# pxl-th/NNop.jl

Hardware: AMD Instinct MI355X
Metric: attention TFLOPs/s + GB/s (fwd, fwd+bwd) at E=64,L=4096,H=4,B=4 (higher is better)
Workload: dtype bf16; 1 GPU; C2: bf16 non-causal flash_attention forward, E=64 L=4096 QH=4 KH=4 B=4 per GPU; per_gpu_batch=4, global_batch=4, parallelism=dp1 over (batch, kv-head) slices, step=one nnop_fa_fwd call

## Files before the change

nnop.jl_amd/_lib.py:

```python
from __future__ import annotations

import ctypes as C
import numbers
import os
import sys

_HERE = os.path.dirname(os.path.abspath(__file__))
LIB_PATH = os.environ.get("NNOP_LIB_PATH") or os.path.join(_HERE, "lib", "libnnop_hip.so")

ABI_VERSION = 7

NNOP_F32, NNOP_F16, NNOP_BF16 = 0, 1, 2

NNOP_OK = 0
NNOP_ERR_EMB_MISMATCH = -1
NNOP_ERR_KV_SHAPE = -2
NNOP_ERR_EMB_NOT_POW2 = -3
NNOP_ERR_HEADS = -4
NNOP_ERR_DTYPE = -5
NNOP_ERR_NULL = -6
NNOP_ERR_EMB_UNSUPPORTED = -7
NNOP_ERR_SHAPE = -8
NNOP_ERR_WORKSPACE = -9
NNOP_ERR_HIP = -10
NNOP_ERR_ALIGN = -11
NNOP_ERR_OPTS = -12

FWD_FORMS = {0: "fa_fwd_kernel", 1: "fa_fwd_split_kernel", 2: "fa_fwd_w64_kernel", 3: "fa_fwd_generic_kernel", 4: "fa_fwd_duo_kernel"}
FWD_FORMS_CAP = {0: "fa_fwd_cap_kernel", 3: "fa_fwd_generic_cap_kernel"}
TUNE_KEYS = {"fwd_split": 0, "fwd_nw": 1, "fwd_w64": 2, "bwd_big7": 3, "norm_bwd_cap": 4, "bwd_nw": 5,
             "fwd_exact_scale": 6, "bwd_w64": 7, "bwd_stages": 8, "fwd_persist": 9, "bwd_persist": 10, "fwd_duo": 11, "fwd_persist_asc": 12, "bwd_narrow": 13, "fwd_causal_alt": 14}


class FaShard(C.Structure):
    """struct nnop_fa_shard (declared below FaDesc; fields filled in after it)"""


class FaDesc(C.Structure):
    _fields_ = [
        ("dtype", C.c_int32), ("emb", C.c_int32), ("ql", C.c_int32), ("kl", C.c_int32),
        ("qh", C.c_int32), ("kh", C.c_int32), ("batch", C.c_int32), ("causal", C.c_int32),
        ("emb_k", C.c_int32), ("emb_v", C.c_int32), ("kl_v", C.c_int32), ("kh_v", C.c_int32),
    ]


FaShard._fields_ = [("desc", FaDesc), ("b0", C.c_int32), ("b1", C.c_int32), ("kh0", C.c_int32), ("kh1", C.c_int32),
# ... 206 lines not shown
```

nnop.jl_amd/csrc/fa_fwd.hpp:

```cpp
#pragma once
#include <type_traits>
#include "fa_common.hpp"

#if !defined(NNOP_DEV_BUILD)
#undef NNOP_ABL
#endif
#ifndef NNOP_ABL
#define NNOP_ABL 0
#endif
#if !defined(NNOP_DEV_BUILD)
#undef NNOP_V_PREFETCH
#undef NNOP_V_DEEP
#undef NNOP_V_MFMASUM
#undef NNOP_V_SETPRIO
#endif
#ifndef NNOP_V_PREFETCH
#define NNOP_V_PREFETCH 1
#endif
#ifndef NNOP_V_DEEP
#define NNOP_V_DEEP 1
#endif
#ifndef NNOP_V_MFMASUM
#define NNOP_V_MFMASUM 1
#endif
// ... 16 lines not shown
    const uint8_t* kpad;
    int   QL, KL, QH, KH, B;
    int   causal;
    int   n_qblk;
    int   n_wg;
    float scale;
    int   persist_hx = 0;
    int   persist = 0;
    int   persist_asc = 0;
    int   causal_alt = 0;
    int   win_left = -1;
    int   win_right = -1;
    const float* sinks = nullptr;
    float cap_ka = 0.f;
    float cap_kb = 0.f;
#ifdef NNOP_DEV_BUILD
    int   stagger = 0;
#endif
};

#include "fa_fwd_kernel.inc"

template <typename T, int E, int BK> constexpr int fa_fwd_lds_bytes() {
    return 2 * (RowImg<T, E>::bytes(BK) + ColImg<T, E>::bytes(BK)) + 16 + 8 * kMaxMaskTiles;
}

}
```

nnop.jl_amd/csrc/fa_fwd_duo_asm.inc:

```
#define NNOP_DUO_SLOTS_PER_GROUP 3
#define NNOP_DUO_VALU_SUMS 0
#define NNOP_DUO_SYNC_ONE 1

#define NNOP_DUO_LOOP_PLAIN(TS, MP1, MP0, VP1, VP0) \
    "v_mov_b32 v208, 0\n\t" \
    "v_mov_b32 v209, 0\n\t" \
    "v_mov_b32 v210, 0xff800000\n\t" \
    "v_mov_b32 v211, 0xff800000\n\t" \
    "s_cmp_lg_u32 %[st], 0\n\t" \
    "s_cbranch_scc1 L_loop1_%=\n\t" \
    "L_loop0_%=:\n\t" \
    "s_cmp_lt_i32 %[st], %[snlive]\n\t" \
    "s_cselect_b32 s56, 1, 0\n\t" \
    "s_sub_i32 s58, %[st], 2\n\t" \
    "s_cmp_lt_i32 s58, %[snlive]\n\t" \
    "s_cselect_b32 s57, 1, 0\n\t" \
    "s_cmp_lt_i32 s58, 0\n\t" \
    "s_cselect_b32 s57, 0, s57\n\t" \
    "v_add_u32 v204, %[ska], v199\n\t" \
    "v_add_u32 v205, %[sva], v200\n\t" \
    "s_add_i32 s58, %[st], 4\n\t" \
    "s_lshl_b32 s58, s58, 13\n\t" \
    "s_min_u32 s60, s58, %[slast]\n\t" \
    "s_add_i32 s58, %[st], 2\n\t" \
// ... 549 lines not shown
    "v_mul_f32 v58, v58, v217\n\t" \
    "v_mul_f32 v59, v59, v217\n\t" \
    "v_mul_f32 v60, v60, v217\n\t" \
    "v_mul_f32 v61, v61, v217\n\t" \
    "v_mul_f32 v62, v62, v217\n\t" \
    "v_mul_f32 v63, v63, v217\n\t" \
    "ds_bpermute_b32 v218, v212, v217\n\t" \
    "ds_bpermute_b32 v219, v213, v217\n\t" \
    "s_waitcnt lgkmcnt(0)\n\t" \
    "v_mul_f32 v100, v100, v218\n\t" \
    "v_mul_f32 v101, v101, v219\n\t" \
    "s_branch L_rescdone0_%=\n\t" \
    "L_exit0_%=:\n\t" \
    "s_branch L_end_%=\n\t" \
    "L_loop1_%=:\n\t" \
    "s_cmp_lt_i32 %[st], %[snlive]\n\t" \
    "s_cselect_b32 s56, 1, 0\n\t" \
    "s_sub_i32 s58, %[st], 2\n\t" \
    "s_cmp_lt_i32 s58, %[snlive]\n\t" \
    "s_cselect_b32 s57, 1, 0\n\t" \
    "s_cmp_lt_i32 s58, 0\n\t" \
    "s_cselect_b32 s57, 0, s57\n\t" \
    "v_add_u32 v204, %[ska], v199\n\t" \
    "v_add_u32 v205, %[sva], v200\n\t" \
    "s_add_i32 s58, %[st], 4\n\t" \
    "s_lshl_b32 s58, s58, 13\n\t" \
    "s_min_u32 s60, s58, %[slast]\n\t" \
    "s_add_i32 s58, %[st], 2\n\t" \
    "s_lshl_b32 s58, s58, 13\n\t" \
    "s_min_u32 s61, s58, %[slast]\n\t" \
// ... 547 lines not shown
    "v_mul_f32 v55, v55, v217\n\t" \
    "v_mul_f32 v56, v56, v217\n\t" \
    "v_mul_f32 v57, v57, v217\n\t" \
    "v_mul_f32 v58, v58, v217\n\t" \
    "v_mul_f32 v59, v59, v217\n\t" \
    "v_mul_f32 v60, v60, v217\n\t" \
    "v_mul_f32 v61, v61, v217\n\t" \
    "v_mul_f32 v62, v62, v217\n\t" \
    "v_mul_f32 v63, v63, v217\n\t" \
    "ds_bpermute_b32 v218, v212, v217\n\t" \
    "ds_bpermute_b32 v219, v213, v217\n\t" \
    "s_waitcnt lgkmcnt(0)\n\t" \
    "v_mul_f32 v100, v100, v218\n\t" \
    "v_mul_f32 v101, v101, v219\n\t" \
    "s_branch L_rescdone1_%=\n\t" \
    "L_exit1_%=:\n\t" \
    "L_end_%=:\n\t"

#define NNOP_DUO_LOOP_MASKED(TS, MP1, MP0, VP1, VP0) \
    "v_mov_b32 v208, 0\n\t" \
    "v_mov_b32 v209, 0\n\t" \
    "v_mov_b32 v210, 0xff800000\n\t" \
    "v_mov_b32 v211, 0xff800000\n\t" \
    "s_cmp_lg_u32 %[st], 0\n\t" \
    "s_cbranch_scc1 L_loop1_%=\n\t" \
    "L_loop0_%=:\n\t" \
    "s_cmp_lt_i32 %[st], %[snlive]\n\t" \
    "s_cselect_b32 s56, 1, 0\n\t" \
    "s_sub_i32 s58, %[st], 2\n\t" \
    "s_cmp_lt_i32 s58, %[snlive]\n\t" \
// ... 7739 lines not shown
    "v_mul_f32 v58, v58, v217\n\t" \
    "v_mul_f32 v59, v59, v217\n\t" \
    "v_mul_f32 v60, v60, v217\n\t" \
    "v_mul_f32 v61, v61, v217\n\t" \
    "v_mul_f32 v62, v62, v217\n\t" \
    "v_mul_f32 v63, v63, v217\n\t" \
    "ds_bpermute_b32 v218, v212, v217\n\t" \
    "ds_bpermute_b32 v219, v213, v217\n\t" \
    "s_waitcnt lgkmcnt(0)\n\t" \
    "v_mul_f32 v100, v100, v218\n\t" \
    "v_mul_f32 v101, v101, v219\n\t" \
    "s_branch L_rescdone0_%=\n\t" \
    "L_exit0_%=:\n\t" \
    "s_branch L_end_%=\n\t" \
    "L_loop1_%=:\n\t" \
    "s_cmp_lt_i32 %[st], %[snlive]\n\t" \
    "s_cselect_b32 s56, 1, 0\n\t" \
    "s_sub_i32 s58, %[st], 2\n\t" \
    "s_cmp_lt_i32 s58, %[snlive]\n\t" \
    "s_cselect_b32 s57, 1, 0\n\t" \
    "s_cmp_lt_i32 s58, 0\n\t" \
    "s_cselect_b32 s57, 0, s57\n\t" \
    "v_add_u32 v204, %[ska], v199\n\t" \
    "v_add_u32 v205, %[sva], v200\n\t" \
    "s_add_i32 s58, %[st], 4\n\t" \
    "s_lshl_b32 s58, s58, 13\n\t" \
    "s_min_u32 s60, s58, %[slast]\n\t" \
    "s_add_i32 s58, %[st], 2\n\t" \
    "s_lshl_b32 s58, s58, 13\n\t" \
    "s_min_u32 s61, s58, %[slast]\n\t" \
// ... 567 lines not shown
    "v_mul_f32 v55, v55, v217\n\t" \
    "v_mul_f32 v56, v56, v217\n\t" \
    "v_mul_f32 v57, v57, v217\n\t" \
    "v_mul_f32 v58, v58, v217\n\t" \
    "v_mul_f32 v59, v59, v217\n\t" \
    "v_mul_f32 v60, v60, v217\n\t" \
    "v_mul_f32 v61, v61, v217\n\t" \
    "v_mul_f32 v62, v62, v217\n\t" \
    "v_mul_f32 v63, v63, v217\n\t" \
    "ds_bpermute_b32 v218, v212, v217\n\t" \
    "ds_bpermute_b32 v219, v213, v217\n\t" \
    "s_waitcnt lgkmcnt(0)\n\t" \
    "v_mul_f32 v100, v100, v218\n\t" \
    "v_mul_f32 v101, v101, v219\n\t" \
    "s_branch L_rescdone1_%=\n\t" \
    "L_exit1_%=:\n\t" \
    "L_end_%=:\n\t" \
    "v_mov_b32 v224, s71\n\t" \
    "v_mov_b32 v225, s72\n\t" \
    "v_mov_b32 v226, s73\n\t" \
    "v_mov_b32 v227, s74\n\t" \
    "v_mov_b32 v228, s75\n\t"

#define NNOP_DUO_LOOP_MASKED_PROF(TS, MP1, MP0, VP1, VP0) \
    "v_mov_b32 v208, 0\n\t" \
    "v_mov_b32 v209, 0\n\t" \
    "v_mov_b32 v210, 0xff800000\n\t" \
    "v_mov_b32 v211, 0xff800000\n\t" \
    "s_memtime s[68:69]\n\t" \
    "s_waitcnt lgkmcnt(0)\n\t" \
// ... 1732 lines not shown
```

nnop.jl_amd/csrc/fa_fwd_duo_kernel.inc:

```
template <typename T, int E, int MODE, int NZ = 2, bool SINK = false>
__global__ __launch_bounds__(512) void fa_fwd_duo_kernel(const FwdParams p) {
    static_assert(sizeof(T) == 2 && ((E == 64 && (NZ == 1 || NZ == 2)) || (E == 128 && NZ == 1) || (E == 32 && NZ == 2)),
                  "16-bit element types; E = 64, E = 128 with 32-row waves, E = 32 with 64-row waves");
    constexpr int RW = 32 * NZ, RB = 4 * RW;
    using frag_t = typename Elem<T>::frag;
    using KImg   = RowImg<T, E>;
    using VImg   = ColImg<T, E>;
    constexpr bool kGeneral = MODE != 0;
    constexpr int BK = 64, KB = 2, KS = E / 16, EB = E / 32, NS = 2 * duo_slots_per_group<E>();
    constexpr int KBYTES = KImg::bytes(BK), VBYTES = VImg::bytes(BK);
    constexpr int RING = NS * (KBYTES + VBYTES);
    constexpr int MASK_OFF = RING > kDuoXchgBytes ? RING : kDuoXchgBytes;
    constexpr int TILE_BYTES = BK * E * (int)sizeof(T);
    constexpr int NJK = KBYTES / 4096, NJV = VBYTES / 4096;
    static_assert(NJK * 4096 == KBYTES && NJV * 4096 == VBYTES && NJK <= 4 && NJV <= 4, "four waves x NJ pieces = one image");

    extern __shared__ __attribute__((aligned(16))) char smem[];
#if NNOP_DUO_STAMP
    uint64_t stamp[8];
    stamp[0] = __builtin_amdgcn_s_memtime();
    stamp[1] = __builtin_amdgcn_s_memrealtime();
#endif
    const int tid = threadIdx.x, lane = tid & 63;
    const int wave = __builtin_amdgcn_readfirstlane(tid >> 6);
// ... 165 lines not shown

    f32x16 sc[NZ][KB];
#pragma unroll
    for (int z = 0; z < NZ; ++z)
#pragma unroll
        for (int kb = 0; kb < KB; ++kb)
#pragma unroll
            for (int i = 0; i < 16; ++i) sc[z][kb][i] = 0.f;

    f32x4 mstate = {-INFINITY, -INFINITY, -INFINITY, -INFINITY};
    typedef uint32_t u32x8 __attribute__((ext_vector_type(8)));
    u32x8 vconst;
    vconst[0] = k_voff[0]; vconst[1] = k_voff[NJK > 1 ? 1 : 0]; vconst[2] = v_voff; vconst[3] = k_lane; vconst[4] = v_lane;
    vconst[5] = (uint32_t)qlim[0]; vconst[6] = (uint32_t)qlim[1]; vconst[7] = (uint32_t)(4 * h);
    int s_t = grp, s_h = n_tiles + 2, s_nlive = n_live, s_cq0 = causal_q0;
    uint32_t s_ka = kA, s_kb = kB, s_kc = kC, s_va = vA, s_vb = vB, s_vc = vC;
    const uint32_t s_last = (uint32_t)(n_tiles - 1) * (uint32_t)TILE_BYTES, s_vbits = (uint32_t)(uintptr_t)vbits;
#if NNOP_DUO_STAMP
    f32x8 profv = {0.f, 0.f, 0.f, 0.f, 0.f, 0.f, 0.f, 0.f};
#endif
#if NNOP_DUO_VALU_SUMS
    f32x4 lsum = {0.f, 0.f, 0.f, 0.f};
#endif
#if NNOP_DUO_PRIO == 2
    if (grp) __builtin_amdgcn_s_setprio(1);
#endif
    if constexpr (!duo_sync_one<E>()) {
        if (grp) asm volatile("s_barrier" ::: "memory");
    }
#if NNOP_DUO_STAMP
// ... 175 lines not shown
```

nnop.jl_amd/csrc/fa_fwd_inst.hpp:

```cpp
#pragma once
#include "fa_fwd.hpp"
#include "fa_fwd_split.hpp"
#include "fa_fwd_w64.hpp"
#include "fa_fwd_duo.hpp"
#include "fa_generic.hpp"
#ifdef NNOP_DEV_BUILD
#include <stdlib.h>
#endif
#include "fa_launch.hpp"
#include <math.h>

namespace nnop {

#ifdef NNOP_DEV_BUILD
static inline int dev_env_int(const char* name, int dflt) {
    const char* s = getenv(name);
    return (s && *s) ? atoi(s) : dflt;
}
#endif

static inline int fwd_params(FwdParams& p, const nnop_fa_desc& d, const FwdArgs& a, int rows) {
    p = FwdParams{};
    p.o = a.o; p.ms = a.ms; p.ls = a.ls;
    p.q = a.q; p.k = a.k; p.v = a.v; p.pair = a.pair; p.kpad = a.kpad;
// ... 89 lines not shown

template <typename T, int E, int MODE, int NZ, bool SINK = false>
static int launch_fwd_duo(const nnop_fa_desc& d, const FwdArgs& a, hipStream_t s) {
    if constexpr (!SINK) {
        if (a.sinks) return launch_fwd_duo<T, E, MODE, NZ, true>(d, a, s);
    }
    constexpr int lds = fa_fwd_duo_lds_bytes<T, E>(MODE != 0);
    static_assert(lds <= 160 * 1024, "LDS budget");
    constexpr auto kern = fa_fwd_duo_kernel<T, E, MODE, NZ, SINK>;
    static unsigned long long lds_done = 0;
    if (ensure_dynamic_lds(kern, lds, &lds_done) != NNOP_OK) return NNOP_ERR_HIP;
    FwdParams p;
    if (const int st = fwd_params(p, d, a, 128 * NZ); st != NNOP_OK) return st;
    long long grid = p.n_wg;
    if constexpr (MODE == 1) fwd_persist_plan(d, a, p, grid);
    hipLaunchKernelGGL(kern, dim3((unsigned)grid), dim3(512), lds, s, p);
    return hipGetLastError() == hipSuccess ? NNOP_OK : NNOP_ERR_HIP;
}

static inline int fwd_mode(const nnop_fa_desc& d, bool has_pair, bool has_mask, bool win_on, bool capped) {
    return has_pair ? 2 : ((d.causal || has_mask || win_on || capped || (d.kl % 64) != 0) ? 1 : 0);
}
static inline long long fwd_wg(const nnop_fa_desc& d, int rows) { return (long long)((d.ql + rows - 1) / rows) * d.qh * d.batch; }
static inline bool fwd_wide_fits(const nnop_fa_desc& d, int mode) {
    return mode != 2 && (mode == 0 || d.kl <= 64 * kMaxMaskTiles) && (long long)d.kl * d.emb * 2 < (1LL << 32);
}
static inline int fwd_duo_nz(const nnop_fa_desc& d) {
    const int duo = tune_get(kTuneFwdDuo);
    if (duo == 2) return 2;
    if (duo == 3) return 1;
// ... 124 lines not shown
```

nnop.jl_amd/csrc/nnop_capi.cpp:

```cpp
#include "fa_launch.hpp"
#include "host_common.hpp"
#include "nnop_debug.h"
#include "tuning.hpp"
#include <limits.h>
#include <stdlib.h>
#include <mutex>

namespace nnop {

static int g_tune[kTuneCount];
static int g_debug_hooks = 0;
static std::once_flag g_tune_once;
static void tune_init() {
    static const char* const names[kTuneCount] = {"NNOP_FWD_SPLIT", "NNOP_FWD_NW",       "NNOP_FWD_W64",
                                                  "NNOP_BWD_BIG7",  "NNOP_NORM_BWD_CAP", "NNOP_BWD_NW",
                                                  "NNOP_FWD_EXACT_SCALE", "NNOP_BWD_W64", nullptr, "NNOP_FWD_PERSIST", "NNOP_BWD_PERSIST",
                                                  "NNOP_FWD_DUO", "NNOP_FWD_PERSIST_ASC", "NNOP_BWD_NARROW", "NNOP_FWD_CAUSAL_ALT"};
    for (int k = 0; k < kTuneCount; ++k) {
        const char* s = names[k] ? getenv(names[k]) : nullptr;
        __atomic_store_n(&g_tune[k], (s && *s) ? atoi(s) : -1, __ATOMIC_RELAXED);
    }
    const char* h = getenv("NNOP_DEBUG_HOOKS");
    __atomic_store_n(&g_debug_hooks, (h && *h && atoi(h) != 0) ? 1 : 0, __ATOMIC_RELAXED);
}
int tune_get(int key) {
    std::call_once(g_tune_once, tune_init);
    return __atomic_load_n(&g_tune[key], __ATOMIC_RELAXED);
}

static int check_desc(const nnop_fa_desc* d) {
    if (!d) return NNOP_ERR_NULL;
    if (!known_dtype(d->dtype)) return NNOP_ERR_DTYPE;
// ... 432 lines not shown
```

nnop.jl_amd/csrc/tuning.hpp:

```cpp
#pragma once

namespace nnop {

enum TuneKey {
    kTuneFwdSplit = 0,
    kTuneFwdNW,
    kTuneFwdW64,
    kTuneBwdBig7,
    kTuneNormBwdCap,
    kTuneBwdNW,
    kTuneFwdExactScale,
    kTuneBwdW64,
    kTuneBwdStages,
    kTuneFwdPersist,
    kTuneBwdPersist,
    kTuneFwdDuo,
    kTuneFwdPersistAsc,
    kTuneBwdNarrow,
    kTuneFwdCausalAlt,
    kTuneCount
};

int tune_get(int key);

}
```

Measured before the change: 1019 TFLOP/s.

## Add unrolled steady-state inner loop to duo forward attention kernel

Adds a specialized steady-state path to the duo forward kernel's main loop. For E=64 with two row groups in the unmasked mode, the loop is unrolled three times with the K/V LDS buffer rotation fixed at compile time. This drops the per-iteration liveness checks, buffer-offset computation and branching of the general loop, and moves the rare online-softmax rescale to out-of-line blocks. It is gated by a new NNOP_FWD_DUO_STEADY knob that is on by default. In exchange it adds a large amount of hand-written asm and a padded rescale path with long s_nop runs, which costs time whenever a rescale is taken.

After: 975.1 TFLOP/s. -4.3%, worse.

```diff
diff --git a/nnop.jl_amd/_lib.py b/nnop.jl_amd/_lib.py
--- a/nnop.jl_amd/_lib.py
+++ b/nnop.jl_amd/_lib.py
@@ -29,7 +29,7 @@
 FWD_FORMS = {0: "fa_fwd_kernel", 1: "fa_fwd_split_kernel", 2: "fa_fwd_w64_kernel", 3: "fa_fwd_generic_kernel", 4: "fa_fwd_duo_kernel"}
 FWD_FORMS_CAP = {0: "fa_fwd_cap_kernel", 3: "fa_fwd_generic_cap_kernel"}
 TUNE_KEYS = {"fwd_split": 0, "fwd_nw": 1, "fwd_w64": 2, "bwd_big7": 3, "norm_bwd_cap": 4, "bwd_nw": 5,
-             "fwd_exact_scale": 6, "bwd_w64": 7, "bwd_stages": 8, "fwd_persist": 9, "bwd_persist": 10, "fwd_duo": 11, "fwd_persist_asc": 12, "bwd_narrow": 13, "fwd_causal_alt": 14}
+             "fwd_exact_scale": 6, "bwd_w64": 7, "bwd_stages": 8, "fwd_persist": 9, "bwd_persist": 10, "fwd_duo": 11, "fwd_persist_asc": 12, "bwd_narrow": 13, "fwd_causal_alt": 14, "fwd_duo_steady": 15}
 
 
 class FaShard(C.Structure):
diff --git a/nnop.jl_amd/csrc/fa_fwd.hpp b/nnop.jl_amd/csrc/fa_fwd.hpp
--- a/nnop.jl_amd/csrc/fa_fwd.hpp
+++ b/nnop.jl_amd/csrc/fa_fwd.hpp
@@ -54,6 +54,7 @@
     const float* sinks = nullptr;
     float cap_ka = 0.f;
     float cap_kb = 0.f;
+    int   duo_steady = 0;
 #ifdef NNOP_DEV_BUILD
     int   stagger = 0;
 #endif
diff --git a/nnop.jl_amd/csrc/fa_fwd_duo_asm.inc b/nnop.jl_amd/csrc/fa_fwd_duo_asm.inc
--- a/nnop.jl_amd/csrc/fa_fwd_duo_asm.inc
+++ b/nnop.jl_amd/csrc/fa_fwd_duo_asm.inc
@@ -1,6 +1,437 @@
 #define NNOP_DUO_SLOTS_PER_GROUP 3
 #define NNOP_DUO_VALU_SUMS 0
 #define NNOP_DUO_SYNC_ONE 1
+
+
+#define NNOP_DUO_STEADY_COPY1(TS, MP1, MP0, VP1, VP0, C, KA, KB, KC, VA, VB, VC, T71, T73, T74, T75) \
+    "v_add_u32 v204, " KA ", v199\n\t" \
+    "v_add_u32 v205, " VA ", v200\n\t" \
+    "" MP1 "\n\t" \
+    "v_xor_b32 v108, 32, v204\n\t" \
+    "v_xor_b32 v109, 64, v204\n\t" \
+    "v_xor_b32 v110, 96, v204\n\t" \
+    "ds_read_b64_tr_b16 v[176:177], v205 offset:0\n\t" \
+    "ds_read_b64_tr_b16 v[178:179], v205 offset:1024\n\t" \
+    "ds_read_b64_tr_b16 v[180:181], v205 offset:256\n\t" \
+    "ds_read_b64_tr_b16 v[182:183], v205 offset:1280\n\t" \
+    "ds_read_b64_tr_b16 v[184:185], v205 offset:2048\n\t" \
+    "ds_read_b64_tr_b16 v[186:187], v205 offset:3072\n\t" \
+    "v_mfma_f32_16x16x32_" TS " v[96:99], v[104:107], v[112:115], v[96:99]\n\t" \
+    "v_mfma_f32_16x16x32_" TS " v[100:103], v[104:107], v[144:147], v[100:103]\n\t" \
+    "v_mfma_f32_16x16x32_" TS " v[96:99], v[104:107], v[120:123], v[96:99]\n\t" \
+    "v_mfma_f32_16x16x32_" TS " v[100:103], v[104:107], v[152:155], v[100:103]\n\t" \
+    "v_mfma_f32_16x16x32_" TS " v[96:99], v[104:107], v[128:131], v[96:99]\n\t" \
+    "v_mfma_f32_16x16x32_" TS " v[100:103], v[104:107], v[160:163], v[100:103]\n\t" \
+    "v_mfma_f32_16x16x32_" TS " v[96:99], v[104:107], v[136:139], v[96:99]\n\t" \
+    "v_mfma_f32_16x16x32_" TS " v[100:103], v[104:107], v[168:171], v[100:103]\n\t" \
+    "ds_read_b64_tr_b16 v[188:189], v205 offset:2304\n\t" \
+    "ds_read_b64_tr_b16 v[190:191], v205 offset:3328\n\t" \
+    "s_waitcnt lgkmcnt(6)\n\t" \
+    "v_mfma_f32_32x32x16_" TS " v[0:15], v[176:179], v[112:115], v[0:15]\n\t" \
+    "v_mfma_f32_32x32x16_" TS " v[32:47], v[176:179], v[144:147], v[32:47]\n\t" \
+    "ds_read_b64_tr_b16 v[176:177], v205 offset:4096\n\t" \
+    "ds_read_b64_tr_b16 v[178:179], v205 offset:5120\n\t" \
+    "s_waitcnt lgkmcnt(6)\n\t" \
+    "v_mfma_f32_32x32x16_" TS " v[16:31], v[180:183], v[112:115], v[16:31]\n\t" \
+    "v_mfma_f32_32x32x16_" TS " v[48:63], v[180:183], v[144:147], v[48:63]\n\t" \
+    "ds_read_b64_tr_b16 v[180:181], v205 offset:4352\n\t" \
+    "ds_read_b64_tr_b16 v[182:183], v205 offset:5376\n\t" \
+    "s_waitcnt lgkmcnt(6)\n\t" \
+    "v_mfma_f32_32x32x16_" TS " v[0:15], v[184:187], v[120:123], v[0:15]\n\t" \
+    "v_mfma_f32_32x32x16_" TS " v[32:47], v[184:187], v[152:155], v[32:47]\n\t" \
+    "ds_read_b64_tr_b16 v[184:185], v205 offset:6144\n\t" \
+    "ds_read_b64_tr_b16 v[186:187], v205 offset:7168\n\t" \
+    "s_waitcnt lgkmcnt(6)\n\t" \
+    "v_mfma_f32_32x32x16_" TS " v[16:31], v[188:191], v[120:123], v[16:31]\n\t" \
+    "v_mfma_f32_32x32x16_" TS " v[48:63], v[188:191], v[152:155], v[48:63]\n\t" \
+    "ds_read_b64_tr_b16 v[188:189], v205 offset:6400\n\t" \
+    "ds_read_b64_tr_b16 v[190:191], v205 offset:7424\n\t" \
+    "s_waitcnt lgkmcnt(6)\n\t" \
+    "v_mfma_f32_32x32x16_" TS " v[0:15], v[176:179], v[128:131], v[0:15]\n\t" \
+    "v_mfma_f32_32x32x16_" TS " v[32:47], v[176:179], v[160:163], v[32:47]\n\t" \
+    "ds_read_b128 v[176:179], v204 offset:0\n\t" \
+    "s_waitcnt lgkmcnt(5)\n\t" \
+    "v_mfma_f32_32x32x16_" TS " v[16:31], v[180:183], v[128:131], v[16:31]\n\t" \
+    "v_mfma_f32_32x32x16_" TS " v[48:63], v[180:183], v[160:163], v[48:63]\n\t" \
+    "ds_read_b128 v[180:183], v108 offset:0\n\t" \
+    "s_waitcnt lgkmcnt(4)\n\t" \
+    "v_mfma_f32_32x32x16_" TS " v[0:15], v[184:187], v[136:139], v[0:15]\n\t" \
+    "v_mfma_f32_32x32x16_" TS " v[32:47], v[184:187], v[168:171], v[32:47]\n\t" \
+    "ds_read_b128 v[184:187], v109 offset:0\n\t" \
+    "s_waitcnt lgkmcnt(3)\n\t" \
+    "v_mfma_f32_32x32x16_" TS " v[16:31], v[188:191], v[136:139], v[16:31]\n\t" \
+    "v_mfma_f32_32x32x16_" TS " v[48:63], v[188:191], v[168:171], v[48:63]\n\t" \
+    "ds_read_b128 v[188:191], v110 offset:0\n\t" \
+    "s_waitcnt lgkmcnt(3)\n\t" \
+    "v_mfma_f32_32x32x16_" TS " v[112:127], v[176:179], v[64:67], 0\n\t" \
+    "v_mfma_f32_32x32x16_" TS " v[144:159], v[176:179], v[80:83], 0\n\t" \
+    "ds_read_b128 v[176:179], v204 offset:4096\n\t" \
+    "s_waitcnt lgkmcnt(3)\n\t" \
+    "v_mfma_f32_32x32x16_" TS " v[112:127], v[180:183], v[68:71], v[112:127]\n\t" \
+    "v_mfma_f32_32x32x16_" TS " v[144:159], v[180:183], v[84:87], v[144:159]\n\t" \
+    "ds_read_b128 v[180:183], v108 offset:4096\n\t" \
+    "s_waitcnt lgkmcnt(3)\n\t" \
+    "v_mfma_f32_32x32x16_" TS " v[112:127], v[184:187], v[72:75], v[112:127]\n\t" \
+    "v_mfma_f32_32x32x16_" TS " v[144:159], v[184:187], v[88:91], v[144:159]\n\t" \
+    "ds_read_b128 v[184:187], v109 offset:4096\n\t" \
+    "s_waitcnt lgkmcnt(3)\n\t" \
+    "v_mfma_f32_32x32x16_" TS " v[112:127], v[188:191], v[76:79], v[112:127]\n\t" \
+    "v_mfma_f32_32x32x16_" TS " v[144:159], v[188:191], v[92:95], v[144:159]\n\t" \
+    "ds_read_b128 v[188:191], v110 offset:4096\n\t" \
+    "s_waitcnt lgkmcnt(3)\n\t" \
+    "v_mfma_f32_32x32x16_" TS " v[128:143], v[176:179], v[64:67], 0\n\t" \
+    "v_mfma_f32_32x32x16_" TS " v[160:175], v[176:179], v[80:83], 0\n\t" \
+    "s_waitcnt lgkmcnt(2)\n\t" \
+    "v_mfma_f32_32x32x16_" TS " v[128:143], v[180:183], v[68:71], v[128:143]\n\t" \
+    "v_mfma_f32_32x32x16_" TS " v[160:175], v[180:183], v[84:87], v[160:175]\n\t" \
+    "s_waitcnt lgkmcnt(1)\n\t" \
+    "v_mfma_f32_32x32x16_" TS " v[128:143], v[184:187], v[72:75], v[128:143]\n\t" \
+    "v_mfma_f32_32x32x16_" TS " v[160:175], v[184:187], v[88:91], v[160:175]\n\t" \
+    "s_waitcnt lgkmcnt(0)\n\t" \
+    "v_mfma_f32_32x32x16_" TS " v[128:143], v[188:191], v[76:79], v[128:143]\n\t" \
+    "v_mfma_f32_32x32x16_" TS " v[160:175], v[188:191], v[92:95], v[160:175]\n\t" \
+    "s_mov_b32 m0, " KC "\n\t" \
+    "s_nop 0\n\t" \
+    "buffer_load_dwordx4 v196, %[krs], s60 offen offset:0 lds\n\t" \
+    "buffer_load_dwordx4 v197, %[krs], s60 offen offset:1024 lds\n\t" \
+    "s_mov_b32 m0, " VC "\n\t" \
+    "s_nop 0\n\t" \
+    "buffer_load_dwordx4 v198, %[vrs], s61 offen offset:0 lds\n\t" \
+    "buffer_load_dwordx4 v198, %[vrs], s61 offen offset:1024 lds\n\t" \
+    "" MP0 "\n\t" \
+    "" T71 "\n\t" \
+    "" T73 "\n\t" \
+    "s_waitcnt vmcnt(4)\n\t" \
+    "" T74 "\n\t" \
+    "s_barrier\n\t" \
+    "" T75 "\n\t" \
+    "" VP1 "\n\t" \
+    "v_max_f32 v176, v112, v113\n\t" \
+    "v_max_f32 v180, v144, v145\n\t" \
+    "v_max_f32 v177, v114, v115\n\t" \
+    "v_max_f32 v181, v146, v147\n\t" \
+    "v_max_f32 v178, v116, v117\n\t" \
+    "v_max_f32 v182, v148, v149\n\t" \
+    "v_max_f32 v179, v118, v119\n\t" \
+    "v_max_f32 v183, v150, v151\n\t" \
+    "v_max3_f32 v176, v176, v120, v121\n\t" \
+    "v_max3_f32 v180, v180, v152, v153\n\t" \
+    "v_max3_f32 v177, v177, v122, v123\n\t" \
+    "v_max3_f32 v181, v181, v154, v155\n\t" \
+    "v_max3_f32 v178, v178, v124, v125\n\t" \
+    "v_max3_f32 v182, v182, v156, v157\n\t" \
+    "v_max3_f32 v179, v179, v126, v127\n\t" \
+    "v_max3_f32 v183, v183, v158, v159\n\t" \
+    "v_max3_f32 v176, v176, v128, v129\n\t" \
+    "v_max3_f32 v180, v180, v160, v161\n\t" \
+    "v_max3_f32 v177, v177, v130, v131\n\t" \
+    "v_max3_f32 v181, v181, v162, v163\n\t" \
+    "v_max3_f32 v178, v178, v132, v133\n\t" \
+    "v_max3_f32 v182, v182, v164, v165\n\t" \
+    "v_max3_f32 v179, v179, v134, v135\n\t" \
+    "v_max3_f32 v183, v183, v166, v167\n\t" \
+    "v_max3_f32 v176, v176, v136, v137\n\t" \
+    "v_max3_f32 v180, v180, v168, v169\n\t" \
+    "v_max3_f32 v177, v177, v138, v139\n\t" \
+    "v_max3_f32 v181, v181, v170, v171\n\t" \
+    "v_max3_f32 v178, v178, v140, v141\n\t" \
+    "v_max3_f32 v182, v182, v172, v173\n\t" \
+    "v_max3_f32 v179, v179, v142, v143\n\t" \
+    "v_max3_f32 v183, v183, v174, v175\n\t" \
+    "v_max3_f32 v176, v176, v177, v178\n\t" \
+    "v_max3_f32 v180, v180, v181, v182\n\t" \
+    "v_max_f32 v206, v176, v179\n\t" \
+    "v_max_f32 v207, v180, v183\n\t" \
+    "v_mul_f32 v206, %[sc2], v206\n\t" \
+    "v_mul_f32 v207, %[sc2], v207\n\t" \
+    "v_max_f32 v194, v194, v206\n\t" \
+    "v_max_f32 v195, v195, v207\n\t" \
+    "v_cmp_gt_f32 vcc, v206, v210\n\t" \
+    "v_cmp_gt_f32 s[64:65], v207, v211\n\t" \
+    "s_or_b64 s[64:65], s[64:65], vcc\n\t" \
+    "s_cbranch_scc1 L_strescale1" C "_%=\n\t" \
+    "L_strescdone1" C "_%=:\n\t" \
+    "v_fma_f32 v112, v112, %[sc2], v208\n\t" \
+    "v_fma_f32 v113, v113, %[sc2], v208\n\t" \
+    "v_fma_f32 v114, v114, %[sc2], v208\n\t" \
+    "v_fma_f32 v115, v115, %[sc2], v208\n\t" \
+    "v_fma_f32 v116, v116, %[sc2], v208\n\t" \
+    "v_exp_f32 v112, v112\n\t" \
+    "v_fma_f32 v117, v117, %[sc2], v208\n\t" \
+    "v_exp_f32 v113, v113\n\t" \
+    "v_fma_f32 v118, v118, %[sc2], v208\n\t" \
+    "v_exp_f32 v114, v114\n\t" \
+    "v_fma_f32 v119, v119, %[sc2], v208\n\t" \
+    "v_exp_f32 v115, v115\n\t" \
+    "v_fma_f32 v144, v144, %[sc2], v209\n\t" \
+    "v_exp_f32 v116, v116\n\t" \
+    "v_fma_f32 v145, v145, %[sc2], v209\n\t" \
+    "v_exp_f32 v117, v117\n\t" \
+    "v_cvt_pk_" TS "_f32 v112, v112, v113\n\t" \
+    "v_fma_f32 v146, v146, %[sc2], v209\n\t" \
+    "v_exp_f32 v118, v118\n\t" \
+    "v_fma_f32 v147, v147, %[sc2], v209\n\t" \
+    "v_exp_f32 v119, v119\n\t" \
+    "v_cvt_pk_" TS "_f32 v113, v114, v115\n\t" \
+    "v_fma_f32 v148, v148, %[sc2], v209\n\t" \
+    "v_exp_f32 v144, v144\n\t" \
+    "v_fma_f32 v149, v149, %[sc2], v209\n\t" \
+    "v_exp_f32 v145, v145\n\t" \
+    "v_cvt_pk_" TS "_f32 v114, v116, v117\n\t" \
+    "v_fma_f32 v150, v150, %[sc2], v209\n\t" \
+    "v_exp_f32 v146, v146\n\t" \
+    "v_fma_f32 v151, v151, %[sc2], v209\n\t" \
+    "v_exp_f32 v147, v147\n\t" \
+    "v_cvt_pk_" TS "_f32 v115, v118, v119\n\t" \
+    "v_fma_f32 v120, v120, %[sc2], v208\n\t" \
+    "v_exp_f32 v148, v148\n\t" \
+    "v_fma_f32 v121, v121, %[sc2], v208\n\t" \
+    "v_exp_f32 v149, v149\n\t" \
+    "v_cvt_pk_" TS "_f32 v144, v144, v145\n\t" \
+    "v_fma_f32 v122, v122, %[sc2], v208\n\t" \
+    "v_exp_f32 v150, v150\n\t" \
+    "v_fma_f32 v123, v123, %[sc2], v208\n\t" \
+    "v_exp_f32 v151, v151\n\t" \
+    "v_cvt_pk_" TS "_f32 v145, v146, v147\n\t" \
+    "v_fma_f32 v124, v124, %[sc2], v208\n\t" \
+    "v_exp_f32 v120, v120\n\t" \
+    "v_fma_f32 v125, v125, %[sc2], v208\n\t" \
+    "v_exp_f32 v121, v121\n\t" \
+    "v_cvt_pk_" TS "_f32 v146, v148, v149\n\t" \
+    "v_fma_f32 v126, v126, %[sc2], v208\n\t" \
+    "v_exp_f32 v122, v122\n\t" \
+    "v_fma_f32 v127, v127, %[sc2], v208\n\t" \
+    "v_exp_f32 v123, v123\n\t" \
+    "v_cvt_pk_" TS "_f32 v147, v150, v151\n\t" \
+    "v_fma_f32 v152, v152, %[sc2], v209\n\t" \
+    "v_exp_f32 v124, v124\n\t" \
+    "v_fma_f32 v153, v153, %[sc2], v209\n\t" \
+    "v_exp_f32 v125, v125\n\t" \
+    "v_cvt_pk_" TS "_f32 v120, v120, v121\n\t" \
+    "v_fma_f32 v154, v154, %[sc2], v209\n\t" \
+    "v_exp_f32 v126, v126\n\t" \
+    "v_fma_f32 v155, v155, %[sc2], v209\n\t" \
+    "v_exp_f32 v127, v127\n\t" \
+    "v_cvt_pk_" TS "_f32 v121, v122, v123\n\t" \
+    "v_fma_f32 v156, v156, %[sc2], v209\n\t" \
+    "v_exp_f32 v152, v152\n\t" \
+    "v_fma_f32 v157, v157, %[sc2], v209\n\t" \
+    "v_exp_f32 v153, v153\n\t" \
+    "v_cvt_pk_" TS "_f32 v122, v124, v125\n\t" \
+    "v_fma_f32 v158, v158, %[sc2], v209\n\t" \
+    "v_exp_f32 v154, v154\n\t" \
+    "v_fma_f32 v159, v159, %[sc2], v209\n\t" \
+    "v_exp_f32 v155, v155\n\t" \
+    "v_cvt_pk_" TS "_f32 v123, v126, v127\n\t" \
+    "v_fma_f32 v128, v128, %[sc2], v208\n\t" \
+    "v_exp_f32 v156, v156\n\t" \
+    "v_fma_f32 v129, v129, %[sc2], v208\n\t" \
+    "v_exp_f32 v157, v157\n\t" \
+    "v_cvt_pk_" TS "_f32 v152, v152, v153\n\t" \
+    "v_fma_f32 v130, v130, %[sc2], v208\n\t" \
+    "v_exp_f32 v158, v158\n\t" \
+    "v_fma_f32 v131, v131, %[sc2], v208\n\t" \
+    "v_exp_f32 v159, v159\n\t" \
+    "v_cvt_pk_" TS "_f32 v153, v154, v155\n\t" \
+    "v_fma_f32 v132, v132, %[sc2], v208\n\t" \
+    "v_exp_f32 v128, v128\n\t" \
+    "v_fma_f32 v133, v133, %[sc2], v208\n\t" \
+    "v_exp_f32 v129, v129\n\t" \
+    "v_cvt_pk_" TS "_f32 v154, v156, v157\n\t" \
+    "v_fma_f32 v134, v134, %[sc2], v208\n\t" \
+    "v_exp_f32 v130, v130\n\t" \
+    "v_fma_f32 v135, v135, %[sc2], v208\n\t" \
+    "v_exp_f32 v131, v131\n\t" \
+    "v_cvt_pk_" TS "_f32 v155, v158, v159\n\t" \
+    "v_fma_f32 v160, v160, %[sc2], v209\n\t" \
+    "v_exp_f32 v132, v132\n\t" \
+    "v_fma_f32 v161, v161, %[sc2], v209\n\t" \
+    "v_exp_f32 v133, v133\n\t" \
+    "v_cvt_pk_" TS "_f32 v128, v128, v129\n\t" \
+    "v_fma_f32 v162, v162, %[sc2], v209\n\t" \
+    "v_exp_f32 v134, v134\n\t" \
+    "v_fma_f32 v163, v163, %[sc2], v209\n\t" \
+    "v_exp_f32 v135, v135\n\t" \
+    "v_cvt_pk_" TS "_f32 v129, v130, v131\n\t" \
+    "v_fma_f32 v164, v164, %[sc2], v209\n\t" \
+    "v_exp_f32 v160, v160\n\t" \
+    "v_fma_f32 v165, v165, %[sc2], v209\n\t" \
+    "v_exp_f32 v161, v161\n\t" \
+    "v_cvt_pk_" TS "_f32 v130, v132, v133\n\t" \
+    "v_fma_f32 v166, v166, %[sc2], v209\n\t" \
+    "v_exp_f32 v162, v162\n\t" \
+    "v_fma_f32 v167, v167, %[sc2], v209\n\t" \
+    "v_exp_f32 v163, v163\n\t" \
+    "v_cvt_pk_" TS "_f32 v131, v134, v135\n\t" \
+    "v_fma_f32 v136, v136, %[sc2], v208\n\t" \
+    "v_exp_f32 v164, v164\n\t" \
+    "v_fma_f32 v137, v137, %[sc2], v208\n\t" \
+    "v_exp_f32 v165, v165\n\t" \
+    "v_cvt_pk_" TS "_f32 v160, v160, v161\n\t" \
+    "v_fma_f32 v138, v138, %[sc2], v208\n\t" \
+    "v_exp_f32 v166, v166\n\t" \
+    "v_fma_f32 v139, v139, %[sc2], v208\n\t" \
+    "v_exp_f32 v167, v167\n\t" \
+    "v_cvt_pk_" TS "_f32 v161, v162, v163\n\t" \
+    "v_fma_f32 v140, v140, %[sc2], v208\n\t" \
+    "v_exp_f32 v136, v136\n\t" \
+    "v_fma_f32 v141, v141, %[sc2], v208\n\t" \
+    "v_exp_f32 v137, v137\n\t" \
+    "v_cvt_pk_" TS "_f32 v162, v164, v165\n\t" \
+    "v_fma_f32 v142, v142, %[sc2], v208\n\t" \
+    "v_exp_f32 v138, v138\n\t" \
+    "v_fma_f32 v143, v143, %[sc2], v208\n\t" \
+    "v_exp_f32 v139, v139\n\t" \
+    "v_cvt_pk_" TS "_f32 v163, v166, v167\n\t" \
+    "v_fma_f32 v168, v168, %[sc2], v209\n\t" \
+    "v_exp_f32 v140, v140\n\t" \
+    "v_fma_f32 v169, v169, %[sc2], v209\n\t" \
+    "v_exp_f32 v141, v141\n\t" \
+    "v_cvt_pk_" TS "_f32 v136, v136, v137\n\t" \
+    "v_fma_f32 v170, v170, %[sc2], v209\n\t" \
+    "v_exp_f32 v142, v142\n\t" \
+    "v_fma_f32 v171, v171, %[sc2], v209\n\t" \
+    "v_exp_f32 v143, v143\n\t" \
+    "v_cvt_pk_" TS "_f32 v137, v138, v139\n\t" \
+    "v_fma_f32 v172, v172, %[sc2], v209\n\t" \
+    "v_exp_f32 v168, v168\n\t" \
+    "v_fma_f32 v173, v173, %[sc2], v209\n\t" \
+    "v_exp_f32 v169, v169\n\t" \
+    "v_cvt_pk_" TS "_f32 v138, v140, v141\n\t" \
+    "v_fma_f32 v174, v174, %[sc2], v209\n\t" \
+    "v_exp_f32 v170, v170\n\t" \
+    "v_fma_f32 v175, v175, %[sc2], v209\n\t" \
+    "v_exp_f32 v171, v171\n\t" \
+    "v_cvt_pk_" TS "_f32 v139, v142, v143\n\t" \
+    "v_exp_f32 v172, v172\n\t" \
+    "v_exp_f32 v173, v173\n\t" \
+    "v_cvt_pk_" TS "_f32 v168, v168, v169\n\t" \
+    "v_exp_f32 v174, v174\n\t" \
+    "v_exp_f32 v175, v175\n\t" \
+    "v_cvt_pk_" TS "_f32 v169, v170, v171\n\t" \
+    "v_cvt_pk_" TS "_f32 v170, v172, v173\n\t" \
+    "v_cvt_pk_" TS "_f32 v171, v174, v175\n\t" \
+    "" VP0 "\n\t" \
+    "s_add_u32 s60, s60, 16384\n\t" \
+    "s_add_u32 s61, s61, 16384\n\t"
+
+#define NNOP_DUO_RESCALE \
+    "s_nop 15\n\t" \
+    "s_nop 15\n\t" \
+    "s_nop 15\n\t" \
+    "s_nop 15\n\t" \
+    "s_nop 15\n\t" \
+    "s_nop 15\n\t" \
+    "s_nop 15\n\t" \
+    "s_nop 15\n\t" \
+    "v_mov_b32 v220, v206\n\t" \
+    "v_mov_b32 v221, v207\n\t" \
+    "s_nop 1\n\t" \
+    "v_permlane32_swap_b32 v206, v220\n\t" \
+    "v_permlane32_swap_b32 v207, v221\n\t" \
+    "v_max_f32 v206, v206, v220\n\t" \
+    "v_max_f32 v207, v207, v221\n\t" \
+    "v_mbcnt_lo_u32_b32 v214, -1, 0\n\t" \
+    "v_mbcnt_hi_u32_b32 v214, -1, v214\n\t" \
+    "v_and_b32 v212, 15, v214\n\t" \
+    "v_lshlrev_b32 v212, 2, v212\n\t" \
+    "v_add_u32 v213, 64, v212\n\t" \
+    "v_cmp_gt_f32 vcc, v206, v210\n\t" \
+    "v_cndmask_b32 v216, v192, v206, vcc\n\t" \
+    "v_sub_f32 v217, v192, v216\n\t" \
+    "v_exp_f32 v217, v217\n\t" \
+    "s_nop 0\n\t" \
+    "v_cndmask_b32 v217, 1.0, v217, vcc\n\t" \
+    "v_mov_b32 v192, v216\n\t" \
+    "v_cmp_eq_f32 vcc, 0xff800000, v216\n\t" \
+    "v_sub_f32 v208, 0, v216\n\t" \
+    "v_cndmask_b32 v208, v208, 0, vcc\n\t" \
+    "v_add_f32 v210, 0x41000000, v216\n\t" \
+    "v_mul_f32 v0, v0, v217\n\t" \
+    "v_mul_f32 v1, v1, v217\n\t" \
+    "v_mul_f32 v2, v2, v217\n\t" \
+    "v_mul_f32 v3, v3, v217\n\t" \
+    "v_mul_f32 v4, v4, v217\n\t" \
+    "v_mul_f32 v5, v5, v217\n\t" \
+    "v_mul_f32 v6, v6, v217\n\t" \
+    "v_mul_f32 v7, v7, v217\n\t" \
+    "v_mul_f32 v8, v8, v217\n\t" \
+    "v_mul_f32 v9, v9, v217\n\t" \
+    "v_mul_f32 v10, v10, v217\n\t" \
+    "v_mul_f32 v11, v11, v217\n\t" \
+    "v_mul_f32 v12, v12, v217\n\t" \
+    "v_mul_f32 v13, v13, v217\n\t" \
+    "v_mul_f32 v14, v14, v217\n\t" \
+    "v_mul_f32 v15, v15, v217\n\t" \
+    "v_mul_f32 v16, v16, v217\n\t" \
+    "v_mul_f32 v17, v17, v217\n\t" \
+    "v_mul_f32 v18, v18, v217\n\t" \
+    "v_mul_f32 v19, v19, v217\n\t" \
+    "v_mul_f32 v20, v20, v217\n\t" \
+    "v_mul_f32 v21, v21, v217\n\t" \
+    "v_mul_f32 v22, v22, v217\n\t" \
+    "v_mul_f32 v23, v23, v217\n\t" \
+    "v_mul_f32 v24, v24, v217\n\t" \
+    "v_mul_f32 v25, v25, v217\n\t" \
+    "v_mul_f32 v26, v26, v217\n\t" \
+    "v_mul_f32 v27, v27, v217\n\t" \
+    "v_mul_f32 v28, v28, v217\n\t" \
+    "v_mul_f32 v29, v29, v217\n\t" \
+    "v_mul_f32 v30, v30, v217\n\t" \
+    "v_mul_f32 v31, v31, v217\n\t" \
+    "ds_bpermute_b32 v218, v212, v217\n\t" \
+    "ds_bpermute_b32 v219, v213, v217\n\t" \
+    "s_waitcnt lgkmcnt(0)\n\t" \
+    "v_mul_f32 v96, v96, v218\n\t" \
+    "v_mul_f32 v97, v97, v219\n\t" \
+    "v_cmp_gt_f32 vcc, v207, v211\n\t" \
+    "v_cndmask_b32 v216, v193, v207, vcc\n\t" \
+    "v_sub_f32 v217, v193, v216\n\t" \
+    "v_exp_f32 v217, v217\n\t" \
+    "s_nop 0\n\t" \
+    "v_cndmask_b32 v217, 1.0, v217, vcc\n\t" \
+    "v_mov_b32 v193, v216\n\t" \
+    "v_cmp_eq_f32 vcc, 0xff800000, v216\n\t" \
+    "v_sub_f32 v209, 0, v216\n\t" \
+    "v_cndmask_b32 v209, v209, 0, vcc\n\t" \
+    "v_add_f32 v211, 0x41000000, v216\n\t" \
+    "v_mul_f32 v32, v32, v217\n\t" \
+    "v_mul_f32 v33, v33, v217\n\t" \
+    "v_mul_f32 v34, v34, v217\n\t" \
+    "v_mul_f32 v35, v35, v217\n\t" \
+    "v_mul_f32 v36, v36, v217\n\t" \
+    "v_mul_f32 v37, v37, v217\n\t" \
+    "v_mul_f32 v38, v38, v217\n\t" \
+    "v_mul_f32 v39, v39, v217\n\t" \
+    "v_mul_f32 v40, v40, v217\n\t" \
+    "v_mul_f32 v41, v41, v217\n\t" \
+    "v_mul_f32 v42, v42, v217\n\t" \
+    "v_mul_f32 v43, v43, v217\n\t" \
+    "v_mul_f32 v44, v44, v217\n\t" \
+    "v_mul_f32 v45, v45, v217\n\t" \
+    "v_mul_f32 v46, v46, v217\n\t" \
+    "v_mul_f32 v47, v47, v217\n\t" \
+    "v_mul_f32 v48, v48, v217\n\t" \
+    "v_mul_f32 v49, v49, v217\n\t" \
+    "v_mul_f32 v50, v50, v217\n\t" \
+    "v_mul_f32 v51, v51, v217\n\t" \
+    "v_mul_f32 v52, v52, v217\n\t" \
+    "v_mul_f32 v53, v53, v217\n\t" \
+    "v_mul_f32 v54, v54, v217\n\t" \
+    "v_mul_f32 v55, v55, v217\n\t" \
+    "v_mul_f32 v56, v56, v217\n\t" \
+    "v_mul_f32 v57, v57, v217\n\t" \
+    "v_mul_f32 v58, v58, v217\n\t" \
+    "v_mul_f32 v59, v59, v217\n\t" \
+    "v_mul_f32 v60, v60, v217\n\t" \
+    "v_mul_f32 v61, v61, v217\n\t" \
+    "v_mul_f32 v62, v62, v217\n\t" \
+    "v_mul_f32 v63, v63, v217\n\t" \
+    "ds_bpermute_b32 v218, v212, v217\n\t" \
+    "ds_bpermute_b32 v219, v213, v217\n\t" \
+    "s_waitcnt lgkmcnt(0)\n\t" \
+    "v_mul_f32 v100, v100, v218\n\t" \
+    "v_mul_f32 v101, v101, v219\n\t"
 
 #define NNOP_DUO_LOOP_PLAIN(TS, MP1, MP0, VP1, VP0) \
     "v_mov_b32 v208, 0\n\t" \
@@ -587,6 +1018,12 @@
     "L_exit0_%=:\n\t" \
     "s_branch L_end_%=\n\t" \
     "L_loop1_%=:\n\t" \
+    "s_cmp_lt_i32 %[st], 2\n\t" \
+    "s_cbranch_scc1 L_general1_%=\n\t" \
+    "s_add_i32 s58, %[st], 11\n\t" \
+    "s_cmp_le_i32 s58, %[scq0]\n\t" \
+    "s_cbranch_scc1 L_steady1_%=\n\t" \
+    "L_general1_%=:\n\t" \
     "s_cmp_lt_i32 %[st], %[snlive]\n\t" \
     "s_cselect_b32 s56, 1, 0\n\t" \
     "s_sub_i32 s58, %[st], 2\n\t" \
@@ -1164,6 +1601,26 @@
     "v_mul_f32 v100, v100, v218\n\t" \
     "v_mul_f32 v101, v101, v219\n\t" \
     "s_branch L_rescdone1_%=\n\t" \
+    "L_steady1_%=:\n\t" \
+    "s_add_i32 s58, %[st], 4\n\t" \
+    "s_lshl_b32 s60, s58, 13\n\t" \
+    "s_add_i32 s58, %[st], 2\n\t" \
+    "s_lshl_b32 s61, s58, 13\n\t" \
+    "L_sttrip1_%=:\n\t" \
+    NNOP_DUO_STEADY_COPY1(TS, MP1, MP0, VP1, VP0, "0", "%[ska]", "%[skb]", "%[skc]", "%[sva]", "%[svb]", "%[svc]", "", "", "", "") \
+    NNOP_DUO_STEADY_COPY1(TS, MP1, MP0, VP1, VP0, "1", "%[skb]", "%[skc]", "%[ska]", "%[svb]", "%[svc]", "%[sva]", "", "", "", "") \
+    NNOP_DUO_STEADY_COPY1(TS, MP1, MP0, VP1, VP0, "2", "%[skc]", "%[ska]", "%[skb]", "%[svc]", "%[sva]", "%[svb]", "", "", "", "") \
+    "s_add_i32 %[st], %[st], 6\n\t" \
+    "s_add_i32 s58, %[st], 11\n\t" \
+    "s_cmp_le_i32 s58, %[scq0]\n\t" \
+    "s_cbranch_scc1 L_sttrip1_%=\n\t" \
+    "s_branch L_loop1_%=\n\t" \
+    "L_strescale10_%=:\n\t" NNOP_DUO_RESCALE \
+    "s_branch L_strescdone10_%=\n\t" \
+    "L_strescale11_%=:\n\t" NNOP_DUO_RESCALE \
+    "s_branch L_strescdone11_%=\n\t" \
+    "L_strescale12_%=:\n\t" NNOP_DUO_RESCALE \
+    "s_branch L_strescdone12_%=\n\t" \
     "L_exit1_%=:\n\t" \
     "L_end_%=:\n\t"
 
@@ -8933,6 +9390,12 @@
     "L_exit0_%=:\n\t" \
     "s_branch L_end_%=\n\t" \
     "L_loop1_%=:\n\t" \
+    "s_cmp_lt_i32 %[st], 2\n\t" \
+    "s_cbranch_scc1 L_general1_%=\n\t" \
+    "s_add_i32 s58, %[st], 11\n\t" \
+    "s_cmp_le_i32 s58, %[scq0]\n\t" \
+    "s_cbranch_scc1 L_steady1_%=\n\t" \
+    "L_general1_%=:\n\t" \
     "s_cmp_lt_i32 %[st], %[snlive]\n\t" \
     "s_cselect_b32 s56, 1, 0\n\t" \
     "s_sub_i32 s58, %[st], 2\n\t" \
@@ -9530,6 +9993,26 @@
     "v_mul_f32 v100, v100, v218\n\t" \
     "v_mul_f32 v101, v101, v219\n\t" \
     "s_branch L_rescdone1_%=\n\t" \
+    "L_steady1_%=:\n\t" \
+    "s_add_i32 s58, %[st], 4\n\t" \
+    "s_lshl_b32 s60, s58, 13\n\t" \
+    "s_add_i32 s58, %[st], 2\n\t" \
+    "s_lshl_b32 s61, s58, 13\n\t" \
+    "L_sttrip1_%=:\n\t" \
+    NNOP_DUO_STEADY_COPY1(TS, MP1, MP0, VP1, VP0, "0", "%[ska]", "%[skb]", "%[skc]", "%[sva]", "%[svb]", "%[svc]", "s_memtime s[68:69]\n\ts_waitcnt lgkmcnt(0)\n\ts_sub_u32 s76, s68, s70\n\ts_add_u32 s71, s71, s76\n\ts_mov_b32 s70, s68", "s_memtime s[68:69]\n\ts_waitcnt lgkmcnt(0)\n\ts_sub_u32 s76, s68, s70\n\ts_add_u32 s73, s73, s76\n\ts_mov_b32 s70, s68", "s_memtime s[68:69]\n\ts_waitcnt lgkmcnt(0)\n\ts_sub_u32 s76, s68, s70\n\ts_add_u32 s74, s74, s76\n\ts_mov_b32 s70, s68", "s_memtime s[68:69]\n\ts_waitcnt lgkmcnt(0)\n\ts_sub_u32 s76, s68, s70\n\ts_add_u32 s75, s75, s76\n\ts_mov_b32 s70, s68") \
+    NNOP_DUO_STEADY_COPY1(TS, MP1, MP0, VP1, VP0, "1", "%[skb]", "%[skc]", "%[ska]", "%[svb]", "%[svc]", "%[sva]", "s_memtime s[68:69]\n\ts_waitcnt lgkmcnt(0)\n\ts_sub_u32 s76, s68, s70\n\ts_add_u32 s71, s71, s76\n\ts_mov_b32 s70, s68", "s_memtime s[68:69]\n\ts_waitcnt lgkmcnt(0)\n\ts_sub_u32 s76, s68, s70\n\ts_add_u32 s73, s73, s76\n\ts_mov_b32 s70, s68", "s_memtime s[68:69]\n\ts_waitcnt lgkmcnt(0)\n\ts_sub_u32 s76, s68, s70\n\ts_add_u32 s74, s74, s76\n\ts_mov_b32 s70, s68", "s_memtime s[68:69]\n\ts_waitcnt lgkmcnt(0)\n\ts_sub_u32 s76, s68, s70\n\ts_add_u32 s75, s75, s76\n\ts_mov_b32 s70, s68") \
+    NNOP_DUO_STEADY_COPY1(TS, MP1, MP0, VP1, VP0, "2", "%[skc]", "%[ska]", "%[skb]", "%[svc]", "%[sva]", "%[svb]", "s_memtime s[68:69]\n\ts_waitcnt lgkmcnt(0)\n\ts_sub_u32 s76, s68, s70\n\ts_add_u32 s71, s71, s76\n\ts_mov_b32 s70, s68", "s_memtime s[68:69]\n\ts_waitcnt lgkmcnt(0)\n\ts_sub_u32 s76, s68, s70\n\ts_add_u32 s73, s73, s76\n\ts_mov_b32 s70, s68", "s_memtime s[68:69]\n\ts_waitcnt lgkmcnt(0)\n\ts_sub_u32 s76, s68, s70\n\ts_add_u32 s74, s74, s76\n\ts_mov_b32 s70, s68", "s_memtime s[68:69]\n\ts_waitcnt lgkmcnt(0)\n\ts_sub_u32 s76, s68, s70\n\ts_add_u32 s75, s75, s76\n\ts_mov_b32 s70, s68") \
+    "s_add_i32 %[st], %[st], 6\n\t" \
+    "s_add_i32 s58, %[st], 11\n\t" \
+    "s_cmp_le_i32 s58, %[scq0]\n\t" \
+    "s_cbranch_scc1 L_sttrip1_%=\n\t" \
+    "s_branch L_loop1_%=\n\t" \
+    "L_strescale10_%=:\n\t" NNOP_DUO_RESCALE \
+    "s_branch L_strescdone10_%=\n\t" \
+    "L_strescale11_%=:\n\t" NNOP_DUO_RESCALE \
+    "s_branch L_strescdone11_%=\n\t" \
+    "L_strescale12_%=:\n\t" NNOP_DUO_RESCALE \
+    "s_branch L_strescdone12_%=\n\t" \
     "L_exit1_%=:\n\t" \
     "L_end_%=:\n\t" \
     "v_mov_b32 v224, s71\n\t" \
diff --git a/nnop.jl_amd/csrc/fa_fwd_duo_kernel.inc b/nnop.jl_amd/csrc/fa_fwd_duo_kernel.inc
--- a/nnop.jl_amd/csrc/fa_fwd_duo_kernel.inc
+++ b/nnop.jl_amd/csrc/fa_fwd_duo_kernel.inc
@@ -203,6 +203,7 @@
     vconst[0] = k_voff[0]; vconst[1] = k_voff[NJK > 1 ? 1 : 0]; vconst[2] = v_voff; vconst[3] = k_lane; vconst[4] = v_lane;
     vconst[5] = (uint32_t)qlim[0]; vconst[6] = (uint32_t)qlim[1]; vconst[7] = (uint32_t)(4 * h);
     int s_t = grp, s_h = n_tiles + 2, s_nlive = n_live, s_cq0 = causal_q0;
+    if constexpr (!kGeneral && E == 64 && NZ == 2) s_cq0 = p.duo_steady ? n_tiles + 2 : 0;
     uint32_t s_ka = kA, s_kb = kB, s_kc = kC, s_va = vA, s_vb = vB, s_vc = vC;
     const uint32_t s_last = (uint32_t)(n_tiles - 1) * (uint32_t)TILE_BYTES, s_vbits = (uint32_t)(uintptr_t)vbits;
 #if NNOP_DUO_STAMP
diff --git a/nnop.jl_amd/csrc/fa_fwd_inst.hpp b/nnop.jl_amd/csrc/fa_fwd_inst.hpp
--- a/nnop.jl_amd/csrc/fa_fwd_inst.hpp
+++ b/nnop.jl_amd/csrc/fa_fwd_inst.hpp
@@ -127,6 +127,7 @@
     if (const int st = fwd_params(p, d, a, 128 * NZ); st != NNOP_OK) return st;
     long long grid = p.n_wg;
     if constexpr (MODE == 1) fwd_persist_plan(d, a, p, grid);
+    if constexpr (MODE == 0 && E == 64 && NZ == 2) p.duo_steady = tune_get(kTuneFwdDuoSteady) != 0 ? 1 : 0;
     hipLaunchKernelGGL(kern, dim3((unsigned)grid), dim3(512), lds, s, p);
     return hipGetLastError() == hipSuccess ? NNOP_OK : NNOP_ERR_HIP;
 }
diff --git a/nnop.jl_amd/csrc/nnop_capi.cpp b/nnop.jl_amd/csrc/nnop_capi.cpp
--- a/nnop.jl_amd/csrc/nnop_capi.cpp
+++ b/nnop.jl_amd/csrc/nnop_capi.cpp
@@ -15,7 +15,8 @@
     static const char* const names[kTuneCount] = {"NNOP_FWD_SPLIT", "NNOP_FWD_NW",       "NNOP_FWD_W64",
                                                   "NNOP_BWD_BIG7",  "NNOP_NORM_BWD_CAP", "NNOP_BWD_NW",
                                                   "NNOP_FWD_EXACT_SCALE", "NNOP_BWD_W64", nullptr, "NNOP_FWD_PERSIST", "NNOP_BWD_PERSIST",
-                                                  "NNOP_FWD_DUO", "NNOP_FWD_PERSIST_ASC", "NNOP_BWD_NARROW", "NNOP_FWD_CAUSAL_ALT"};
+                                                  "NNOP_FWD_DUO", "NNOP_FWD_PERSIST_ASC", "NNOP_BWD_NARROW", "NNOP_FWD_CAUSAL_ALT",
+                                                  "NNOP_FWD_DUO_STEADY"};
     for (int k = 0; k < kTuneCount; ++k) {
         const char* s = names[k] ? getenv(names[k]) : nullptr;
         __atomic_store_n(&g_tune[k], (s && *s) ? atoi(s) : -1, __ATOMIC_RELAXED);
diff --git a/nnop.jl_amd/csrc/tuning.hpp b/nnop.jl_amd/csrc/tuning.hpp
--- a/nnop.jl_amd/csrc/tuning.hpp
+++ b/nnop.jl_amd/csrc/tuning.hpp
@@ -18,6 +18,7 @@
     kTuneFwdPersistAsc,
     kTuneBwdNarrow,
     kTuneFwdCausalAlt,
+    kTuneFwdDuoSteady,
     kTuneCount
 };
 
```
